# julius-speech/julius

Hardware: AMD Instinct MI355X
Metric: frames_x_states_scored_per_sec (higher is better)
Workload: dtype f32; 1 GPU; C2 = configs[1]: triphone GMM outprob only, S=3000 M=16 D=39, step = 12 launches x 64000 frames; frames_per_launch=64000, parallelism=utterance-sharded x1, kernel=gmm_tile<D=39,FPL=2,NS=16,ring> grid=23504 nsb=16

## Files before the change

### julius_amd/csrc/gmm_api.hip

```cpp
#include "gmm_host.h"

extern "C" {

int jamd_gmm_create(jamd_engine *e, const jamd_gmm_desc *d, int gprune, int gprune_num, jamd_gmm **out) {
  if (!e || !d || !out) { jamd_set_error("jamd_gmm_create: NULL argument"); return JAMD_EINVAL; }
  *out = nullptr;
  if (d->nstream != 1) {
    jamd_set_error("jamd_gmm_create: nstream=%d; only single-stream models are supported", d->nstream);
    return JAMD_EINVAL;
  }
  if (d->nstate <= 0 || d->veclen <= 0 || d->veclen > 1024 || d->nentry < 0 || d->ndens < 0) {
    jamd_set_error("jamd_gmm_create: bad dimensions S=%d D=%d G=%d E=%d", d->nstate, d->veclen,
                   d->ndens, d->nentry);
    return JAMD_EINVAL;
  }
  if (gprune != JAMD_GPRUNE_NONE && gprune != JAMD_GPRUNE_SAFE && gprune != JAMD_GPRUNE_HEU && gprune != JAMD_GPRUNE_BEAM) {
    jamd_set_error("jamd_gmm_create: unknown gprune method %d", gprune);
    return JAMD_EINVAL;
  }
  const bool history_pruning = gprune == JAMD_GPRUNE_HEU || gprune == JAMD_GPRUNE_BEAM;
  const int requested_gprune = gprune;
  if (history_pruning) gprune = JAMD_GPRUNE_SAFE;
  if (!d->mean || !d->ivar || !d->gconst || !d->st_off || (d->nentry && (!d->ent_dens || !d->ent_logw))) {
    jamd_set_error("jamd_gmm_create: NULL model array");
    return JAMD_EINVAL;
  }
  if (d->st_off[0] != 0 || d->st_off[d->nstate] != d->nentry) {
    jamd_set_error("jamd_gmm_create: st_off must run from 0 to nentry");
    return JAMD_EINVAL;
  }
  JAMD_HIP(hipSetDevice(e->device));
  std::unique_ptr<jamd_gmm> g(new jamd_gmm());
  int rc;
  g->eng = e; g->S = d->nstate; g->D = d->veclen; g->E = d->nentry;
  g->gprune = gprune; g->gprune_num = gprune_num;
  const int D = g->D;
  g->rec = ((2 * D + 2) + 3) & ~3;
  const bool have_books = d->nbook > 0 && d->st_book;
  std::vector<int> st_off_plain(g->S + 1, 0), tied;
  std::vector<int> book_first(d->nbook > 0 ? d->nbook : 0, -1);
  for (int s = 0; s < g->S; s++) {
    const int n = d->st_off[s + 1] - d->st_off[s];
    if (n < 0) { jamd_set_error("jamd_gmm_create: st_off not monotone at %d", s); return JAMD_EINVAL; }
    const int b = have_books ? d->st_book[s] : -1;
    if (b >= d->nbook) { jamd_set_error("jamd_gmm_create: codebook id %d out of range", b); return JAMD_EINVAL; }
    if (b >= 0) {
      tied.push_back(s);
      if (book_first[b] < 0) book_first[b] = s;
      else if (n != d->st_off[book_first[b] + 1] - d->st_off[book_first[b]]) {
        jamd_set_error("jamd_gmm_create: states of codebook %d disagree on its size", b); return JAMD_EINVAL;
      }
      st_off_plain[s + 1] = st_off_plain[s];
    } else {
      if (n > g->maxmix) g->maxmix = n;
      st_off_plain[s + 1] = st_off_plain[s] + n;
    }
  }
  g->E_plain = st_off_plain[g->S];
  g->ntied = (int)tied.size();
  if (history_pruning && g->ntied > 0) g->hist_method = requested_gprune;
  g->nbook = g->ntied ? d->nbook : 0;
  if (gprune == JAMD_GPRUNE_SAFE && gprune_num < 1) {
    jamd_set_error("jamd_gmm_create: gprune safe needs gprune_num >= 1"); return JAMD_EINVAL;
  }
  if (gprune == JAMD_GPRUNE_SAFE && gprune_num > 64) {
    jamd_set_error("jamd_gmm_create: gprune_num %d > 64 is not supported on the device", gprune_num);
    return JAMD_EINVAL;
  }
  auto fill_rec = [&](float *r, int dn, float lw) -> bool {
    if (dn >= d->ndens) return false;
    if (dn >= 0) {
      memcpy(r, d->mean + (size_t)dn * D, sizeof(float) * D);
      memcpy(r + D, d->ivar + (size_t)dn * D, sizeof(float) * D);
      r[2 * D] = d->gconst[dn];
      if (r[2 * D] != r[2 * D]) g->has_null = true;
    } else {
      r[2 * D] = __builtin_nanf("");
      g->has_null = true;
    }
    r[2 * D + 1] = lw;
    return true;
  };
  std::vector<float> rec((size_t)g->E_plain * g->rec, 0.0f);
  for (int s = 0; s < g->S; s++) {
    if (have_books && d->st_book[s] >= 0) continue;
    for (int k = 0; k < d->st_off[s + 1] - d->st_off[s]; k++) {
      const int en = d->st_off[s] + k;
      if (!fill_rec(rec.data() + (size_t)(st_off_plain[s] + k) * g->rec, d->ent_dens[en], d->ent_logw[en])) {
        jamd_set_error("jamd_gmm_create: density index %d out of range", d->ent_dens[en]); return JAMD_EINVAL;
      }
    }
  }
  if ((rc = g->d_rec.upload(rec.data(), rec.size())) != JAMD_OK) return rc;
  if (D == 39) {
    constexpr int kRing = 80;
    std::vector<float> ring((size_t)g->E_plain * kRing, 0.0f);
    for (int en = 0; en < g->E_plain; en++) {
      const float *r = rec.data() + (size_t)en * g->rec;
      float *q = ring.data() + (size_t)en * kRing;
      q[0] = r[2 * D]; q[1] = r[2 * D + 1];
      for (int k = 0; k < 7; k++) { q[2 + k] = r[k]; q[9 + k] = r[D + k]; }
      for (int c = 1; c < 5; c++)
        for (int k = 0; k < 8; k++) { q[16 * c + k] = r[8 * c - 1 + k]; q[16 * c + 8 + k] = r[D + 8 * c - 1 + k]; }
    }
    if ((rc = g->d_rec_ring.upload(ring.data(), ring.size())) != JAMD_OK) return rc;
  }
  if ((rc = g->d_st_off.upload(d->st_off, g->S + 1)) != JAMD_OK) return rc;
  if ((rc = g->d_st_off_plain.upload(st_off_plain.data(), g->S + 1)) != JAMD_OK) return rc;
  if (g->ntied) {
    std::vector<int> book_off(g->nbook + 1, 0);
    for (int b = 0; b < g->nbook; b++) {
      const int n = book_first[b] >= 0 ? d->st_off[book_first[b] + 1] - d->st_off[book_first[b]] : 0;
      book_off[b + 1] = book_off[b] + n;
      if (n > g->maxbook) g->maxbook = n;
    }
    std::vector<float> brec((size_t)book_off[g->nbook] * g->rec, 0.0f);
    for (int b = 0; b < g->nbook; b++) {
      if (book_first[b] < 0) continue;
      for (int k = 0; k < book_off[b + 1] - book_off[b]; k++) {
        if (!fill_rec(brec.data() + (size_t)(book_off[b] + k) * g->rec,
                      d->ent_dens[d->st_off[book_first[b]] + k], 0.0f)) {
          jamd_set_error("jamd_gmm_create: codebook density index out of range"); return JAMD_EINVAL;
        }
      }
    }
    g->tm_cap = (gprune == JAMD_GPRUNE_NONE) ? g->maxbook : (gprune_num < g->maxbook ? gprune_num : g->maxbook);
    g->h_book_off = book_off;
    if ((rc = g->d_book_rec.upload(brec.data(), brec.size())) != JAMD_OK) return rc;
    if ((rc = g->d_book_off.upload(book_off.data(), g->nbook + 1)) != JAMD_OK) return rc;
    if ((rc = g->d_st_book.upload(d->st_book, g->S)) != JAMD_OK) return rc;
    if ((rc = g->d_ent_logw.upload(d->ent_logw, g->E)) != JAMD_OK) return rc;
    if ((rc = g->d_tied_states.upload(tied.data(), g->ntied)) != JAMD_OK) return rc;
  }
  *out = g.release();
  return JAMD_OK;
}

void jamd_gmm_destroy(jamd_gmm *g) {
  if (!g) return;
  (void)hipSetDevice(g->eng->device);
  delete g;
}

int jamd_gmm_nstate(const jamd_gmm *g) { return g ? g->S : -1; }
int jamd_gmm_veclen(const jamd_gmm *g) { return g ? g->D : -1; }
const char *jamd_gmm_last_kernel(const jamd_gmm *g) { return g ? g->last_kernel : ""; }

int jamd_gmm_nentry(const jamd_gmm *g) {
  if (!g) return 0;
  if (g->ntied == 0) return g->E;
  if (g->ntied == g->S && !g->h_book_off.empty()) return g->h_book_off[g->nbook];
  return 0;
}

int jamd_gmm_book_offsets(const jamd_gmm *g, int *off, int cap) {
  if (!g || !off || g->ntied != g->S || (int)g->h_book_off.size() != g->nbook + 1 || cap < g->nbook + 1) {
    jamd_set_error("jamd_gmm_book_offsets: not an all-tied-mixture model, or buffer too small"); return JAMD_EINVAL;
  }
  memcpy(off, g->h_book_off.data(), sizeof(int) * (size_t)(g->nbook + 1));
  return JAMD_OK;
}

int jamd_gmm_dens_dev(jamd_gmm *g, const float *dev_frames, int T, float *dev_out, void *stream) {
  if (!g || !dev_frames || !dev_out || T < 0) { jamd_set_error("jamd_gmm_dens_dev: bad argument"); return JAMD_EINVAL; }
  const int E = jamd_gmm_nentry(g);
  if (E <= 0) {
    jamd_set_error("jamd_gmm_dens_dev: models mixing plain and tied-mixture states have no single column order");
    return JAMD_EINVAL;
  }
  if (T == 0) return JAMD_OK;
  JAMD_HIP(hipSetDevice(g->eng->device));
  hipStream_t st = jamd_stream(g->eng, stream);
  const int rc = jamd_gmm_launch_dens(g, g->ntied ? g->d_book_rec : g->d_rec, E, dev_frames, T, dev_out, st);
  if (rc != JAMD_OK) return rc;
  hipError_t le = hipGetLastError();
  if (le != hipSuccess) { jamd_set_error("jamd_gmm_dens_dev: launch failed: %s", hipGetErrorString(le)); return JAMD_ELAUNCH; }
  return JAMD_OK;
}

int jamd_gmm_dens_host(jamd_gmm *g, const float *host_frames, int T, float *host_out) {
  if (!g || !host_frames || !host_out || T < 0) { jamd_set_error("jamd_gmm_dens_host: bad argument"); return JAMD_EINVAL; }
  if (T == 0) return JAMD_OK;
  JAMD_HIP(hipSetDevice(g->eng->device));
  const int E = jamd_gmm_nentry(g);
  if (E <= 0) { jamd_set_error("jamd_gmm_dens_host: no single column order for this model"); return JAMD_EINVAL; }
  return jamd_host_call(&g->dens_stage, g->eng, host_frames, (size_t)T * g->D, host_out, (size_t)T * E,
                        [&](const float *in, float *o, hipStream_t st) -> long long {
                          const int rc = jamd_gmm_dens_dev(g, in, T, o, st);
                          return rc != JAMD_OK ? rc : (long long)T * E;
                        }, JAMD_ELAUNCH);
}

static int set_utterances(jamd_gmm *g, const int *utt_off, int nutt, hipStream_t st) {
  if (g->ntied == 0 || g->gprune == JAMD_GPRUNE_NONE) return JAMD_OK;
  const size_t bytes = sizeof(int) * ((size_t)nutt + 1);
  int rc;
  if ((rc = g->utt.begin(bytes < 4096 ? 4096 : bytes)) != JAMD_OK) return rc;
  memcpy(g->utt.h.p, utt_off, bytes);
  if ((rc = g->utt.send(bytes, st)) != JAMD_OK) return rc;
  g->cur_nutt = nutt;
  return JAMD_OK;
}

int jamd_gmm_outprob_dev(jamd_gmm *g, const float *dev_frames, int T, float *dev_out, void *stream) {
  const int off[2] = {0, T};
  if (T < 0) { jamd_set_error("jamd_gmm_outprob_dev: bad argument"); return JAMD_EINVAL; }
  return jamd_gmm_outprob_utts_dev(g, dev_frames, off, 1, dev_out, stream);
}

int jamd_gmm_outprob_utts_dev(jamd_gmm *g, const float *dev_frames, const int *utt_off, int nutt, float *dev_out, void *stream) {
  if (!g || !dev_frames || !dev_out || !utt_off || nutt < 1 || utt_off[0] != 0) {
    jamd_set_error("jamd_gmm_outprob_utts_dev: bad argument");
    return JAMD_EINVAL;
  }
  for (int u = 0; u < nutt; u++)
    if (utt_off[u + 1] < utt_off[u]) { jamd_set_error("jamd_gmm_outprob_utts_dev: utt_off must be non-decreasing"); return JAMD_EINVAL; }
  const int T = utt_off[nutt];
  if (T == 0) return JAMD_OK;
  JAMD_HIP(hipSetDevice(g->eng->device));
  hipStream_t st = jamd_stream(g->eng, stream);
  int rc = JAMD_OK;
  if ((rc = set_utterances(g, utt_off, nutt, st)) != JAMD_OK) return rc;
  if (g->E_plain == 0 && g->ntied == g->S) {
  } else if (g->gprune == JAMD_GPRUNE_SAFE) {
    rc = jamd_gmm_launch_safe(g, dev_frames, T, dev_out, st);
  } else {
    rc = jamd_gmm_launch_plain(g, dev_frames, T, dev_out, st);
  }
  if (rc != JAMD_OK) return rc;
  if (g->ntied) {
    const size_t n = (size_t)T * g->nbook * g->tm_cap;
    if ((rc = g->d_tm_score.grow(sizeof(float) * n)) != JAMD_OK) return rc;
    if ((rc = g->d_tm_id.grow(sizeof(int) * n)) != JAMD_OK) return rc;
    if ((rc = g->d_tm_num.grow(sizeof(int) * (size_t)T * g->nbook)) != JAMD_OK) return rc;
    if ((rc = jamd_gmm_launch_tmix(g, dev_frames, T, dev_out, g->d_tm_score, g->d_tm_id, g->d_tm_num, st)) != JAMD_OK) return rc;
  }
  hipError_t le = hipGetLastError();
  if (le != hipSuccess) {
    jamd_set_error("jamd_gmm_outprob_dev: launch failed: %s", hipGetErrorString(le));
    return JAMD_ELAUNCH;
  }
  return JAMD_OK;
}

int jamd_gmm_outprob_host(jamd_gmm *g, const float *host_frames, int T, float *host_out) {
  if (!g || !host_frames || !host_out || T < 0) {
    jamd_set_error("jamd_gmm_outprob_host: bad argument");
    return JAMD_EINVAL;
  }
  if (T == 0) return JAMD_OK;
  return jamd_host_call(&g->stage, g->eng, host_frames, (size_t)T * g->D, host_out, (size_t)T * g->S,
                        [&](const float *in, float *o, hipStream_t st) -> long long {
                          const int rc = jamd_gmm_outprob_dev(g, in, T, o, st);
                          return rc != JAMD_OK ? rc : (long long)T * g->S;
                        }, JAMD_ELAUNCH);
}

int jamd_gmm_tmix_cap(const jamd_gmm *g) { return g ? g->tm_cap : -1; }
int jamd_gmm_nbook(const jamd_gmm *g) { return g ? g->nbook : -1; }

int jamd_gmm_tmix_cache_dev(jamd_gmm *g, const float *dev_frames, int T, float *dev_score,
                            int *dev_id, int *dev_num, void *stream) {
  if (!g || !dev_frames || !dev_score || !dev_id || !dev_num || T < 0) {
    jamd_set_error("jamd_gmm_tmix_cache_dev: bad argument");
    return JAMD_EINVAL;
  }
  if (!g->ntied) { jamd_set_error("jamd_gmm_tmix_cache_dev: model has no tied-mixture states"); return JAMD_ESTATE; }
  if (T == 0) return JAMD_OK;
  JAMD_HIP(hipSetDevice(g->eng->device));
  const int off[2] = {0, T};
  int rc = set_utterances(g, off, 1, jamd_stream(g->eng, stream));
  if (rc == JAMD_OK) rc = jamd_gmm_launch_tmix(g, dev_frames, T, nullptr, dev_score, dev_id, dev_num, jamd_stream(g->eng, stream));
  if (rc != JAMD_OK) return rc;
  hipError_t le = hipGetLastError();
  if (le != hipSuccess) {
    jamd_set_error("jamd_gmm_tmix_cache_dev: launch failed: %s", hipGetErrorString(le));
    return JAMD_ELAUNCH;
  }
  return JAMD_OK;
}

}
```

### julius_amd/csrc/gmm_host.h

```cpp
#pragma once
#include "jamd_host.h"

struct JAMD_LOCAL jamd_gmm {
  jamd_engine *eng = nullptr;
  int S = 0, D = 0, E = 0, nbook = 0;
  int gprune = 0, gprune_num = 0;
  int rec = 0;
  int maxmix = 0;
  JamdDev<float> d_rec;
  JamdDev<float> d_rec_ring;
  JamdDev<int> d_st_off;
  JamdDev<int> d_st_off_plain;
  int E_plain = 0;
  JamdDev<int> d_st_book;
  JamdDev<int> d_book_off;
  std::vector<int> h_book_off;
  JamdDev<float> d_book_rec;
  JamdDev<float> d_ent_logw;
  JamdDev<int> d_tied_states;
  int ntied = 0;
  int maxbook = 0;
  int tm_cap = 0;
  bool has_null = false;
  int hist_method = 0;
  JamdPinned utt;
  int cur_nutt = 0;
  JamdStage<float, float> stage;
  JamdStage<float, float> dens_stage;
  JamdDev<float> d_tm_score; JamdDev<int> d_tm_id, d_tm_num;
  JamdDev<float> d_narrow;
  JamdDev<int> d_tm_flag;
  char last_kernel[64] = {0};
};

JAMD_LOCAL int jamd_gmm_launch_plain(jamd_gmm *g, const float *frames, int T, float *out, hipStream_t st);
JAMD_LOCAL int jamd_gmm_launch_dens(jamd_gmm *g, const float *rec, int E, const float *frames, int T, float *out,
                                        hipStream_t st);

int jamd_gmm_launch_safe(jamd_gmm *g, const float *frames, int T, float *out, hipStream_t st);
int jamd_gmm_launch_tmix(jamd_gmm *g, const float *frames, int T, float *out, float *c_score,
                         int *c_id, int *c_num, hipStream_t st);
```

### julius_amd/csrc/gmm_outprob.hip

```cpp
#include "gmm_dev.h"
#include "gmm_host.h"

namespace {
using namespace jamd;

constexpr int kWaves = 4;

template <int D, int FPL, int NS, bool HAS_NULL>
__global__ void __launch_bounds__(64 * kWaves)
gmm_tile_kernel(const float *__restrict__ rec, const int *__restrict__ st_off,
                const float *__restrict__ frames, const float *__restrict__ tbl,
                float *__restrict__ out, int T, int S, int nsb, int nfb, int nstb,
                float addmin_f) {
  static_assert(FPL % 2 == 0, "frames are processed as packed pairs");
  constexpr int REC = ((2 * D + 2) + 3) & ~3;
  constexpr int FPW = 64 * FPL;
  constexpr int NP = FPL / 2;
  __shared__ float tile[kWaves][FPW][NS + 1];

  int fb, sb;
  if (!decode_block(nfb, nstb, fb, sb)) return;
  const int lane = threadIdx.x & 63;
  const int wave = threadIdx.x >> 6;
  const int t0 = (fb * kWaves + wave) * FPW;
  if (t0 >= T) return;

  f2 v[NP][D];
#pragma unroll
  for (int p = 0; p < NP; p++) load_frames<D>(v[p], nullptr, frames, t0 + p * 128, T, D, lane);

#if defined(__HIP_DEVICE_COMPILE__) && !defined(__GFX9__)
#error "gmm_tile: the raw buffer descriptor below is the gfx9 (CDNA) format; this library is written for gfx950 only"
#endif
  const __amdgpu_buffer_rsrc_t tbl_rsrc = __builtin_amdgcn_make_buffer_rsrc((void *)tbl, 0, 4 * (JAMD_TBLSIZE + 1), 0x00020000);
  const int s_begin = sb * nsb;
  const int s_end = min(S, s_begin + nsb);
  for (int sg = s_begin; sg < s_end; sg += NS) {
    const int ns = min(NS, s_end - sg);
    for (int si = 0; si < ns; si++) {
      const int e0 = st_off[sg + si], e1 = st_off[sg + si + 1];
      f2 y2[NP], tv2[NP];
#pragma unroll
      for (int p = 0; p < NP; p++) { y2[p] = f2{JAMD_LOG_ZERO, JAMD_LOG_ZERO}; tv2[p] = f2{0.0f, 0.0f}; }
      for (int e = e1 - 1; e >= e0; e--) {
        const float *__restrict__ r = rec + (size_t)e * REC;
        const float gc = r[2 * D], lw = r[2 * D + 1];
        f2 acc[NP];
#pragma unroll
        for (int p = 0; p < NP; p++) acc[p] = f2{gc, gc};
#pragma unroll
        for (int d = 0; d < D; d++) {
          const float mu = r[d], iv = r[D + d];
          const f2 mu2 = {mu, mu}, iv2 = {iv, iv};
#pragma unroll
          for (int p = 0; p < NP; p++) {
            f2 x = v[p][d] - mu2;
            x = x * x;
            x = x * iv2;
            acc[p] = acc[p] + x;
          }
        }
        const bool nulld = HAS_NULL && (gc != gc);
        const float naddmin = -addmin_f;
#pragma unroll
        for (int p = 0; p < NP; p++) {
          f2 s2 = acc[p] * f2{-0.5f, -0.5f};
          if (nulld) s2 = f2{JAMD_LOG_ZERO, JAMD_LOG_ZERO};
          s2 = s2 + f2{lw, lw};
          __builtin_amdgcn_sched_barrier(0);
          const f2 yy = y2[p] + tv2[p];
          const f2 hi = {__builtin_fmaxf(s2.x, yy.x), __builtin_fmaxf(s2.y, yy.y)};
          const f2 df = s2 - yy;
          const float a0 = __builtin_fabsf(df.x), a1 = __builtin_fabsf(df.y);
          unsigned o0 = ((unsigned)((double)a0 * JAMD_TMAG + 0.5)) << 2, o1 = ((unsigned)((double)a1 * JAMD_TMAG + 0.5)) << 2;
          o0 = (a0 <= naddmin) ? o0 : 4u * (unsigned)JAMD_TBLSIZE;
          o1 = (a1 <= naddmin) ? o1 : 4u * (unsigned)JAMD_TBLSIZE;
          tv2[p] = f2{__builtin_bit_cast(float, __builtin_amdgcn_raw_buffer_load_b32(tbl_rsrc, (int)o0, 0, 0)),
                      __builtin_bit_cast(float, __builtin_amdgcn_raw_buffer_load_b32(tbl_rsrc, (int)o1, 0, 0))};
          y2[p] = hi;
        }
      }
#pragma unroll
      for (int k = 0; k < FPL; k++) {
        const f2 fin = y2[k / 2] + tv2[k / 2];
        tile[wave][k * 64 + lane][si] = finish_state((k & 1) ? fin.y : fin.x);
      }
    }
    wave_sync();
    constexpr int RPI = 64 / NS;
    const int col = lane % NS, rsub = lane / NS;
#pragma unroll 4
    for (int it = 0; it < FPW / RPI; it++) {
      const int rr = it * RPI + rsub;
      const int t = t0 + rr;
      if (t < T && col < ns) out[(size_t)t * S + sg + col] = tile[wave][rr][col];
    }
    wave_release();
  }
}

typedef float f16v __attribute__((ext_vector_type(16)));
constexpr int kRingRec = 80;

template <int BYTE_OFF>
__device__ __forceinline__ void ring_load(f16v &home, const float *chunks) {
  __builtin_amdgcn_sched_barrier(0);
  asm volatile("s_load_dwordx16 %0, %1, %2" : "=s"(home) : "s"(chunks), "i"(BYTE_OFF));
  __builtin_amdgcn_sched_barrier(0);
}
__device__ __forceinline__ void ring_wait(f16v &h0, f16v &h1, f16v &h2) {
  __builtin_amdgcn_sched_barrier(0);
  asm volatile("s_waitcnt lgkmcnt(0)" : "+s"(h0), "+s"(h1), "+s"(h2));
  __builtin_amdgcn_sched_barrier(0);
}
template <int N, int MU0, int IV0>
__device__ __forceinline__ void ring_chunk(f2 &acc, const f2 *v, const f16v &h) {
  f2 x[N], q[N], w[N];
#pragma unroll
  for (int i = 0; i < N + 3; i++) {
    if (i < N) { const float mu = h[MU0 + i]; x[i] = v[i] - f2{mu, mu}; }
    if (i >= 1 && i - 1 < N) q[i - 1] = x[i - 1] * x[i - 1];
    if (i >= 2 && i - 2 < N) { const float iv = h[IV0 + i - 2]; w[i - 2] = q[i - 2] * f2{iv, iv}; }
    if (i >= 3) acc = acc + w[i - 3];
    __builtin_amdgcn_sched_barrier(0);
  }
}

template <int NS, bool HAS_NULL>
__global__ void __launch_bounds__(64 * kWaves)
gmm_tile_ring_kernel(const float *__restrict__ ring, const int *__restrict__ st_off,
                     const float *__restrict__ frames, const float *__restrict__ tbl,
                     float *__restrict__ out, int T, int S, int nsb, int nfb, int nstb,
                     float addmin_f) {
  constexpr int D = 39, FPL = 2;
  constexpr int FPW = 64 * FPL;
  __shared__ float tile[kWaves][FPW][NS + 1];

  int fb, sb;
  if (!decode_block(nfb, nstb, fb, sb)) return;
  const int lane = threadIdx.x & 63;
  const int wave = threadIdx.x >> 6;
  const int t0 = (fb * kWaves + wave) * FPW;
  if (t0 >= T) return;

  f2 v[D];
  load_frames<D>(v, nullptr, frames, t0, T, D, lane);

  const __amdgpu_buffer_rsrc_t tbl_rsrc = __builtin_amdgcn_make_buffer_rsrc((void *)tbl, 0, 4 * (JAMD_TBLSIZE + 1), 0x00020000);
  const float naddmin = -addmin_f;
  const int s_begin = sb * nsb;
  const int s_end = min(S, s_begin + nsb);
  f16v h0, h1, h2;
  int held = -1;
  for (int sg = s_begin; sg < s_end; sg += NS) {
    const int ns = min(NS, s_end - sg);
    for (int si = 0; si < ns; si++) {
      const int s = sg + si;
      const int e0 = st_off[s], e1 = st_off[s + 1];
      const int e_over = (s + 1 < s_end ? st_off[s + 2] : e1) - 1;
      f2 y2 = {JAMD_LOG_ZERO, JAMD_LOG_ZERO}, tv2 = {0.0f, 0.0f};
      if (e1 > e0 && held != e1 - 1) {
        const float *r = ring + (size_t)(e1 - 1) * kRingRec;
        ring_load<0>(h0, r);
        ring_load<64>(h1, r);
        ring_load<128>(h2, r);
        ring_wait(h0, h1, h2);
      }
      for (int e = e1 - 1; e >= e0; e--) {
        const float *r = ring + (size_t)e * kRingRec;
        const float *rn = ring + (size_t)(e > e0 ? e - 1 : e_over) * kRingRec;
        const float gc = h0[0], lw = h0[1];
        const bool nulld = HAS_NULL && (gc != gc);
        f2 acc = {gc, gc};
        ring_chunk<7, 2, 9>(acc, v, h0);
        ring_load<192>(h0, r);
        ring_chunk<8, 0, 8>(acc, v + 7, h1);
        ring_load<256>(h1, r);
        ring_chunk<8, 0, 8>(acc, v + 15, h2);
        ring_wait(h0, h1, h2);
        ring_chunk<8, 0, 8>(acc, v + 23, h0);
        ring_load<0>(h0, rn);
        ring_load<128>(h2, rn);
        ring_chunk<8, 0, 8>(acc, v + 31, h1);
        ring_load<64>(h1, rn);
        {
          f2 s2 = acc * f2{-0.5f, -0.5f};
          if (nulld) s2 = f2{JAMD_LOG_ZERO, JAMD_LOG_ZERO};
          s2 = s2 + f2{lw, lw};
          __builtin_amdgcn_sched_barrier(0);
          const f2 yy = y2 + tv2;
          const f2 hi = {__builtin_fmaxf(s2.x, yy.x), __builtin_fmaxf(s2.y, yy.y)};
          const f2 df = s2 - yy;
          const float a0 = __builtin_fabsf(df.x), a1 = __builtin_fabsf(df.y);
          unsigned o0 = ((unsigned)((double)a0 * JAMD_TMAG + 0.5)) << 2, o1 = ((unsigned)((double)a1 * JAMD_TMAG + 0.5)) << 2;
          o0 = (a0 <= naddmin) ? o0 : 4u * (unsigned)JAMD_TBLSIZE;
          o1 = (a1 <= naddmin) ? o1 : 4u * (unsigned)JAMD_TBLSIZE;
          tv2 = f2{__builtin_bit_cast(float, __builtin_amdgcn_raw_buffer_load_b32(tbl_rsrc, (int)o0, 0, 0)),
                   __builtin_bit_cast(float, __builtin_amdgcn_raw_buffer_load_b32(tbl_rsrc, (int)o1, 0, 0))};
          y2 = hi;
        }
        ring_wait(h0, h1, h2);
      }
      if (e1 > e0) held = e_over;
      const f2 fin = y2 + tv2;
      tile[wave][lane][si] = finish_state(fin.x);
      tile[wave][64 + lane][si] = finish_state(fin.y);
    }
    store_tile<NS, FPW>(tile[wave], out, t0, T, S, sg, ns, lane);
  }
}

template <int FPL, int NS>
__global__ void __launch_bounds__(64 * kWaves)
gmm_tile_generic_kernel(const float *__restrict__ rec, const int *__restrict__ st_off,
                        const float *__restrict__ frames, const float *__restrict__ tbl,
                        float *__restrict__ out, int T, int S, int D, int REC, int nsb, int nfb,
                        int nstb, float addmin_f) {
  static_assert(FPL == 2, "load_frames / gauss_pair hold one packed pair of frames per lane");
  constexpr int FPW = 64 * FPL;
  __shared__ float tile[kWaves][FPW][NS + 1];
  extern __shared__ __align__(16) float dyn[];

  int fb, sb;
  if (!decode_block(nfb, nstb, fb, sb)) return;
  const int lane = threadIdx.x & 63;
  const int wave = threadIdx.x >> 6;
  const int t0 = (fb * kWaves + wave) * FPW;
  if (t0 >= T) return;
  float *vt = dyn + (size_t)wave * D * FPW;
  load_frames<0>(nullptr, vt, frames, t0, T, D, lane);

  const int s_begin = sb * nsb;
  const int s_end = min(S, s_begin + nsb);
  for (int sg = s_begin; sg < s_end; sg += NS) {
    const int ns = min(NS, s_end - sg);
    for (int si = 0; si < ns; si++) {
      const int e0 = st_off[sg + si], e1 = st_off[sg + si + 1];
      float y0 = JAMD_LOG_ZERO, y1 = JAMD_LOG_ZERO;
      for (int e = e1 - 1; e >= e0; e--) {
        const float *__restrict__ r = rec + (size_t)e * REC;
        const float lw = r[2 * D + 1];
        const f2 g = gauss_pair<0>(nullptr, vt, lane, D, r);
        y0 = addlog_step(y0, g.x + lw, tbl, addmin_f);
        y1 = addlog_step(y1, g.y + lw, tbl, addmin_f);
      }
      tile[wave][lane][si] = finish_state(y0);
      tile[wave][64 + lane][si] = finish_state(y1);
    }
    store_tile<NS, FPW>(tile[wave], out, t0, T, S, sg, ns, lane);
  }
}

template <int D, int FPL, int NS>
int launch_tile(jamd_gmm *g, const float *frames, int T, float *out, hipStream_t st) {
  constexpr int FPB = kWaves * 64 * FPL;
  const int nfb = (T + FPB - 1) / FPB;
  const int nsb = NS;
  const int nstb = (g->S + nsb - 1) / nsb;
  const int grid = xcd_grid(nstb, nfb);
  if constexpr (D == 39 && FPL == 2) {
    if (g->has_null)
      hipLaunchKernelGGL((gmm_tile_ring_kernel<NS, true>), dim3(grid), dim3(64 * kWaves), 0, st,
                         g->d_rec_ring, g->d_st_off_plain, frames, g->eng->d_addlog, out, T, g->S, nsb, nfb,
                         nstb, g->eng->addmin_f);
    else
      hipLaunchKernelGGL((gmm_tile_ring_kernel<NS, false>), dim3(grid), dim3(64 * kWaves), 0, st,
                         g->d_rec_ring, g->d_st_off_plain, frames, g->eng->d_addlog, out, T, g->S, nsb, nfb,
                         nstb, g->eng->addmin_f);
    snprintf(g->last_kernel, sizeof(g->last_kernel), "gmm_tile<D=%d,FPL=%d,NS=%d,ring> grid=%d nsb=%d", D, FPL, NS, grid, nsb);
  } else {
    if (g->has_null)
      hipLaunchKernelGGL((gmm_tile_kernel<D, FPL, NS, true>), dim3(grid), dim3(64 * kWaves), 0, st,
                         g->d_rec, g->d_st_off_plain, frames, g->eng->d_addlog, out, T, g->S, nsb, nfb,
                         nstb, g->eng->addmin_f);
    else
      hipLaunchKernelGGL((gmm_tile_kernel<D, FPL, NS, false>), dim3(grid), dim3(64 * kWaves), 0, st,
                         g->d_rec, g->d_st_off_plain, frames, g->eng->d_addlog, out, T, g->S, nsb, nfb,
                         nstb, g->eng->addmin_f);
    snprintf(g->last_kernel, sizeof(g->last_kernel), "gmm_tile<D=%d,FPL=%d,NS=%d> grid=%d nsb=%d", D, FPL, NS, grid, nsb);
  }
  return JAMD_OK;
}

template <int FPL, int NS>
int launch_tile_generic(jamd_gmm *g, const float *frames, int T, float *out, hipStream_t st) {
  constexpr int FPB = kWaves * 64 * FPL;
  const int nfb = (T + FPB - 1) / FPB;
  const int nsb = NS;
  const int nstb = (g->S + nsb - 1) / nsb;
  const int grid = xcd_grid(nstb, nfb);
  const size_t dyn = sizeof(float) * kWaves * g->D * 64 * FPL;
  const int rc = jamd_reserve_dyn_lds((const void *)gmm_tile_generic_kernel<FPL, NS>, dyn, "GMM outprob");
  if (rc != JAMD_OK) return rc;
  hipLaunchKernelGGL((gmm_tile_generic_kernel<FPL, NS>), dim3(grid), dim3(64 * kWaves), dyn, st,
                     g->d_rec, g->d_st_off_plain, frames, g->eng->d_addlog, out, T, g->S, g->D, g->rec,
                     nsb, nfb, nstb, g->eng->addmin_f);
  snprintf(g->last_kernel, sizeof(g->last_kernel), "gmm_tile_generic<FPL=%d,NS=%d> D=%d grid=%d",
           FPL, NS, g->D, grid);
  return JAMD_OK;
}

constexpr int kNarrowT = 256;
constexpr int kNarrowFB = 8;
template <int D, bool HAS_NULL>
__global__ void __launch_bounds__(64)
gmm_narrow_dens_kernel(const float *__restrict__ rec, const float *__restrict__ frames, float *__restrict__ dens, int T, int E,
                       int nfb, int neb) {
  constexpr int REC = (2 * D + 2 + 3) & ~3;
  int fbk, ebk;
  if (!decode_block(nfb, neb, fbk, ebk)) return;
  const int e = ebk * 64 + threadIdx.x;
  const float4 *__restrict__ r4 = reinterpret_cast<const float4 *>(rec + (size_t)(e < E ? e : E - 1) * REC);
  float r[REC];
#pragma unroll
  for (int q = 0; q < REC / 4; q++) { const float4 v = r4[q]; r[4 * q] = v.x; r[4 * q + 1] = v.y; r[4 * q + 2] = v.z; r[4 * q + 3] = v.w; }
  const float gc = r[2 * D], lw = r[2 * D + 1];
  const bool nulld = HAS_NULL && (gc != gc);
  const int t_end = min(T, (fbk + 1) * kNarrowFB);
  for (int t = fbk * kNarrowFB; t < t_end; t += 2) {
    const float *__restrict__ fa = frames + (size_t)t * D;
    const float *__restrict__ fb = frames + (size_t)(t + 1 < T ? t + 1 : t) * D;
    f2 acc = {gc, gc};
#pragma unroll
    for (int d = 0; d < D; d++) {
      f2 x = f2{fa[d], fb[d]} - f2{r[d], r[d]};
      x = x * x;
      x = x * f2{r[D + d], r[D + d]};
      acc = acc + x;
    }
    f2 s2 = acc * f2{-0.5f, -0.5f};
    if (nulld) s2 = f2{JAMD_LOG_ZERO, JAMD_LOG_ZERO};
    s2 = s2 + f2{lw, lw};
    if (e < E) {
      dens[(size_t)t * E + e] = s2.x;
      if (t + 1 < T) dens[(size_t)(t + 1) * E + e] = s2.y;
    }
  }
}

__global__ void __launch_bounds__(256)
gmm_narrow_lse_kernel(const float *__restrict__ dens, const int *__restrict__ st_off, const float *__restrict__ tbl,
                      float *__restrict__ out, int T, int S, int E, float addmin_f) {
  const int i = blockIdx.x * 256 + threadIdx.x;
  if (i >= T * S) return;
  const int t = i / S, s = i - t * S;
  const int e0 = st_off[s], e1 = st_off[s + 1];
  const float *__restrict__ dr = dens + (size_t)t * E;
  float y = JAMD_LOG_ZERO;
  int e = e1 - 1;
  for (; e - 7 >= e0; e -= 8) {
    float v[8];
#pragma unroll
    for (int q = 0; q < 8; q++) v[q] = dr[e - q];
#pragma unroll
    for (int q = 0; q < 8; q++) y = addlog_step(y, v[q], tbl, addmin_f);
  }
  for (; e >= e0; e--) y = addlog_step(y, dr[e], tbl, addmin_f);
  out[(size_t)t * S + s] = finish_state(y);
}

template <int D>
int launch_narrow(jamd_gmm *g, const float *frames, int T, float *out, hipStream_t st) {
  const int E = g->E_plain;
  int rc = g->d_narrow.grow(sizeof(float) * (size_t)kNarrowT * (size_t)E);
  if (rc != JAMD_OK) return rc;
  const int grid = (E + 63) / 64;
  const int nfb = (T + kNarrowFB - 1) / kNarrowFB;
  const dim3 gr(xcd_grid(grid, nfb));
  if (g->has_null) hipLaunchKernelGGL((gmm_narrow_dens_kernel<D, true>), gr, dim3(64), 0, st, g->d_rec, frames, g->d_narrow, T, E, nfb, grid);
  else hipLaunchKernelGGL((gmm_narrow_dens_kernel<D, false>), gr, dim3(64), 0, st, g->d_rec, frames, g->d_narrow, T, E, nfb, grid);
  hipLaunchKernelGGL(gmm_narrow_lse_kernel, dim3((T * g->S + 255) / 256), dim3(256), 0, st, g->d_narrow, g->d_st_off_plain,
                     g->eng->d_addlog, out, T, g->S, E, g->eng->addmin_f);
  snprintf(g->last_kernel, sizeof(g->last_kernel), "gmm_narrow<D=%d> grid=%d + lse", D, grid);
  return JAMD_OK;
}

constexpr int kDensChunk = 1024;
__global__ void __launch_bounds__(64)
gmm_dens_kernel(const float *__restrict__ rec, const float *__restrict__ frames, float *__restrict__ out,
                int T, int E, int D, int REC) {
  extern __shared__ float xs[];
  float (*tile)[17] = reinterpret_cast<float (*)[17]>(xs + (size_t)D * 64);
  const int lane = threadIdx.x;
  const int t0 = blockIdx.x * 64, e_begin = blockIdx.y * kDensChunk;
  const int e_end = min(E, e_begin + kDensChunk);
  {
    int t = t0 + lane; if (t > T - 1) t = T - 1;
    const float *f = frames + (size_t)t * D;
    for (int d = 0; d < D; d++) xs[d * 64 + lane] = f[d];
  }
  wave_sync();
  for (int e0 = e_begin; e0 < e_end; e0 += 16) {
    const int ne = min(16, e_end - e0);
    for (int g = 0; g < ne; g++) {
      const float *__restrict__ r = rec + (size_t)(e0 + g) * REC;
      const float gc = r[2 * D];
      float acc = gc;
      for (int d = 0; d < D; d++) {
        float x = xs[d * 64 + lane] - r[d];
        x = x * x;
        x = x * r[D + d];
        acc = acc + x;
      }
      float sc = acc * -0.5f;
      if (gc != gc) sc = JAMD_LOG_ZERO;
      tile[lane][g] = sc;
    }
    wave_sync();
    const int col = lane & 15, rsub = lane >> 4;
    for (int it = 0; it < 16; it++) {
      const int rr = it * 4 + rsub, t = t0 + rr;
      if (t < T && col < ne) out[(size_t)t * E + e0 + col] = tile[rr][col];
    }
    wave_release();
  }
}

}


int jamd_gmm_launch_plain(jamd_gmm *g, const float *frames, int T, float *out, hipStream_t st) {
  const bool narrow = T <= kNarrowT && g->E_plain > 0;
  return dispatch_veclen(g->D, [&](auto dt) {
    constexpr int D = decltype(dt)::value;
    if constexpr (D == 0) return launch_tile_generic<2, 16>(g, frames, T, out, st);
    else return narrow ? launch_narrow<D>(g, frames, T, out, st) : launch_tile<D, 2, 16>(g, frames, T, out, st);
  });
}

int jamd_gmm_launch_dens(jamd_gmm *g, const float *rec, int E, const float *frames, int T, float *out, hipStream_t st) {
  const size_t lds = sizeof(float) * ((size_t)g->D * 64 + 64 * 17);
  if (lds > 64 * 1024) { jamd_set_error("jamd_gmm_dens_dev: vector length %d too large", g->D); return JAMD_EINVAL; }
  hipLaunchKernelGGL(gmm_dens_kernel, dim3((T + 63) / 64, (E + kDensChunk - 1) / kDensChunk), dim3(64), lds, st,
                     rec, frames, out, T, E, g->D, g->rec);
  return JAMD_OK;
}
```

Before: 19.78 billion frame*states/s.

## Add persistent pull-based work distribution to the D=39 ring GMM kernel

Adds a persistent variant of the ring GMM tile kernel. It launches roughly one occupancy-sized grid instead of one block per tile. Each wave pulls (state-range, frame-group) tickets from eight atomic counters spread across cache lines, using a deal that keeps state-range locality per share. The aim is to cut block launch and tail-imbalance overhead on large launches, at the cost of per-ticket atomics, a memset before each launch and reloading frames per ticket. The path is chosen when the tile count exceeds a multiple of the pull grid capacity, and environment variables can override that threshold and the grid size.

```diff
diff --git a/julius_amd/csrc/gmm_api.hip b/julius_amd/csrc/gmm_api.hip
--- a/julius_amd/csrc/gmm_api.hip
+++ b/julius_amd/csrc/gmm_api.hip
@@ -104,6 +104,7 @@
         for (int k = 0; k < 8; k++) { q[16 * c + k] = r[8 * c - 1 + k]; q[16 * c + 8 + k] = r[D + 8 * c - 1 + k]; }
     }
     if ((rc = g->d_rec_ring.upload(ring.data(), ring.size())) != JAMD_OK) return rc;
+    if ((rc = jamd_gmm_pull_setup(g.get())) != JAMD_OK) return rc;
   }
   if ((rc = g->d_st_off.upload(d->st_off, g->S + 1)) != JAMD_OK) return rc;
   if ((rc = g->d_st_off_plain.upload(st_off_plain.data(), g->S + 1)) != JAMD_OK) return rc;
diff --git a/julius_amd/csrc/gmm_deal.h b/julius_amd/csrc/gmm_deal.h
--- /dev/null
+++ b/julius_amd/csrc/gmm_deal.h
@@ -0,0 +1,57 @@
+#pragma once
+
+#if defined(__HIPCC__)
+#define GD_HD __host__ __device__ inline __attribute__((always_inline))
+#else
+#define GD_HD inline
+#endif
+
+constexpr int kGdShares = 8;
+constexpr int kGdHeadStride = 32;
+
+struct GmmDeal {
+  int nfw;
+  int k8;
+  int full;
+  int L, per;
+};
+
+GD_HD GmmDeal gd_make(int nstb, int nfw) {
+  GmmDeal d;
+  d.nfw = nfw;
+  d.k8 = nstb & ~7;
+  d.full = (d.k8 >> 3) * nfw;
+  d.L = (nstb - d.k8) * nfw;
+  d.per = (d.L + 7) >> 3;
+  return d;
+}
+
+GD_HD int gd_len(const GmmDeal &d, int x) {
+  int left = d.L - x * d.per;
+  if (left < 0) left = 0;
+  if (left > d.per) left = d.per;
+  return d.full + left;
+}
+
+GD_HD bool gd_ticket(const GmmDeal &d, int x, int n, int &range, int &group) {
+  if (n < 0) return false;
+  if (n < d.full) {
+    const int q = n / d.nfw;
+    range = x + 8 * q;
+    group = n - q * d.nfw;
+    return true;
+  }
+  const int k = n - d.full;
+  if (k >= d.per) return false;
+  const int m = x * d.per + k;
+  if (m >= d.L) return false;
+  const int q = m / d.nfw;
+  range = d.k8 + q;
+  group = m - q * d.nfw;
+  return true;
+}
+
+GD_HD int gd_pull_grid(int cap, int want) {
+  int g = (want > 0 ? want : cap) & ~7;
+  return g < 8 ? 8 : g;
+}
diff --git a/julius_amd/csrc/gmm_host.h b/julius_amd/csrc/gmm_host.h
--- a/julius_amd/csrc/gmm_host.h
+++ b/julius_amd/csrc/gmm_host.h
@@ -30,10 +30,15 @@
   JamdDev<float> d_tm_score; JamdDev<int> d_tm_id, d_tm_num;
   JamdDev<float> d_narrow;
   JamdDev<int> d_tm_flag;
+  JamdDev<int> d_pull_heads;
+  int pull_cap = 0;
+  int pull_min = 0;
+  int pull_grid = 0;
   char last_kernel[64] = {0};
 };
 
 JAMD_LOCAL int jamd_gmm_launch_plain(jamd_gmm *g, const float *frames, int T, float *out, hipStream_t st);
+JAMD_LOCAL int jamd_gmm_pull_setup(jamd_gmm *g);
 JAMD_LOCAL int jamd_gmm_launch_dens(jamd_gmm *g, const float *rec, int E, const float *frames, int T, float *out,
                                         hipStream_t st);
 
diff --git a/julius_amd/csrc/gmm_outprob.hip b/julius_amd/csrc/gmm_outprob.hip
--- a/julius_amd/csrc/gmm_outprob.hip
+++ b/julius_amd/csrc/gmm_outprob.hip
@@ -1,5 +1,6 @@
 #include "gmm_dev.h"
 #include "gmm_host.h"
+#include "gmm_deal.h"
 
 namespace {
 using namespace jamd;
@@ -126,87 +127,110 @@
   }
 }
 
-template <int NS, bool HAS_NULL>
+template <int NS, bool HAS_NULL, bool PULL>
 __global__ void __launch_bounds__(64 * kWaves)
 gmm_tile_ring_kernel(const float *__restrict__ ring, const int *__restrict__ st_off,
                      const float *__restrict__ frames, const float *__restrict__ tbl,
                      float *__restrict__ out, int T, int S, int nsb, int nfb, int nstb,
-                     float addmin_f) {
+                     float addmin_f, int *__restrict__ heads) {
   constexpr int D = 39, FPL = 2;
   constexpr int FPW = 64 * FPL;
   __shared__ float tile[kWaves][FPW][NS + 1];
 
-  int fb, sb;
-  if (!decode_block(nfb, nstb, fb, sb)) return;
   const int lane = threadIdx.x & 63;
   const int wave = threadIdx.x >> 6;
-  const int t0 = (fb * kWaves + wave) * FPW;
-  if (t0 >= T) return;
-
   f2 v[D];
-  load_frames<D>(v, nullptr, frames, t0, T, D, lane);
+  int sb, t0;
+  if constexpr (!PULL) {
+    int fb;
+    if (!decode_block(nfb, nstb, fb, sb)) return;
+    t0 = (fb * kWaves + wave) * FPW;
+    if (t0 >= T) return;
+    load_frames<D>(v, nullptr, frames, t0, T, D, lane);
+  }
 
   const __amdgpu_buffer_rsrc_t tbl_rsrc = __builtin_amdgcn_make_buffer_rsrc((void *)tbl, 0, 4 * (JAMD_TBLSIZE + 1), 0x00020000);
   const float naddmin = -addmin_f;
-  const int s_begin = sb * nsb;
-  const int s_end = min(S, s_begin + nsb);
+  int share = blockIdx.x & (kGdShares - 1), spent = 0;
   f16v h0, h1, h2;
   int held = -1;
-  for (int sg = s_begin; sg < s_end; sg += NS) {
-    const int ns = min(NS, s_end - sg);
-    for (int si = 0; si < ns; si++) {
-      const int s = sg + si;
-      const int e0 = st_off[s], e1 = st_off[s + 1];
-      const int e_over = (s + 1 < s_end ? st_off[s + 2] : e1) - 1;
-      f2 y2 = {JAMD_LOG_ZERO, JAMD_LOG_ZERO}, tv2 = {0.0f, 0.0f};
-      if (e1 > e0 && held != e1 - 1) {
-        const float *r = ring + (size_t)(e1 - 1) * kRingRec;
-        ring_load<0>(h0, r);
-        ring_load<64>(h1, r);
-        ring_load<128>(h2, r);
-        ring_wait(h0, h1, h2);
-      }
-      for (int e = e1 - 1; e >= e0; e--) {
-        const float *r = ring + (size_t)e * kRingRec;
-        const float *rn = ring + (size_t)(e > e0 ? e - 1 : e_over) * kRingRec;
-        const float gc = h0[0], lw = h0[1];
-        const bool nulld = HAS_NULL && (gc != gc);
-        f2 acc = {gc, gc};
-        ring_chunk<7, 2, 9>(acc, v, h0);
-        ring_load<192>(h0, r);
-        ring_chunk<8, 0, 8>(acc, v + 7, h1);
-        ring_load<256>(h1, r);
-        ring_chunk<8, 0, 8>(acc, v + 15, h2);
-        ring_wait(h0, h1, h2);
-        ring_chunk<8, 0, 8>(acc, v + 23, h0);
-        ring_load<0>(h0, rn);
-        ring_load<128>(h2, rn);
-        ring_chunk<8, 0, 8>(acc, v + 31, h1);
-        ring_load<64>(h1, rn);
-        {
-          f2 s2 = acc * f2{-0.5f, -0.5f};
-          if (nulld) s2 = f2{JAMD_LOG_ZERO, JAMD_LOG_ZERO};
-          s2 = s2 + f2{lw, lw};
-          __builtin_amdgcn_sched_barrier(0);
-          const f2 yy = y2 + tv2;
-          const f2 hi = {__builtin_fmaxf(s2.x, yy.x), __builtin_fmaxf(s2.y, yy.y)};
-          const f2 df = s2 - yy;
-          const float a0 = __builtin_fabsf(df.x), a1 = __builtin_fabsf(df.y);
-          unsigned o0 = ((unsigned)((double)a0 * JAMD_TMAG + 0.5)) << 2, o1 = ((unsigned)((double)a1 * JAMD_TMAG + 0.5)) << 2;
-          o0 = (a0 <= naddmin) ? o0 : 4u * (unsigned)JAMD_TBLSIZE;
-          o1 = (a1 <= naddmin) ? o1 : 4u * (unsigned)JAMD_TBLSIZE;
-          tv2 = f2{__builtin_bit_cast(float, __builtin_amdgcn_raw_buffer_load_b32(tbl_rsrc, (int)o0, 0, 0)),
-                   __builtin_bit_cast(float, __builtin_amdgcn_raw_buffer_load_b32(tbl_rsrc, (int)o1, 0, 0))};
-          y2 = hi;
+  for (;;) {
+    if constexpr (PULL) {
+      const GmmDeal deal = gd_make(nstb, nfb);
+      int group = 0;
+      bool got = false;
+      while (spent < kGdShares) {
+        int n = 0;
+        if (lane == 0) n = __hip_atomic_fetch_add(heads + share * kGdHeadStride, 1, __ATOMIC_RELAXED, __HIP_MEMORY_SCOPE_AGENT);
+        n = __builtin_amdgcn_readfirstlane(n);
+        got = gd_ticket(deal, share, n, sb, group);
+        if (got) break;
+        share = (share + 1) & (kGdShares - 1);
+        spent++;
+      }
+      if (!got) return;
+      t0 = group * FPW;
+      load_frames<D>(v, nullptr, frames, t0, T, D, lane);
+    }
+    const int s_begin = sb * nsb;
+    const int s_end = min(S, s_begin + nsb);
+    for (int sg = s_begin; sg < s_end; sg += NS) {
+      const int ns = min(NS, s_end - sg);
+      for (int si = 0; si < ns; si++) {
+        const int s = sg + si;
+        const int e0 = st_off[s], e1 = st_off[s + 1];
+        const int e_over = (s + 1 < s_end ? st_off[s + 2] : e1) - 1;
+        f2 y2 = {JAMD_LOG_ZERO, JAMD_LOG_ZERO}, tv2 = {0.0f, 0.0f};
+        if (e1 > e0 && held != e1 - 1) {
+          const float *r = ring + (size_t)(e1 - 1) * kRingRec;
+          ring_load<0>(h0, r);
+          ring_load<64>(h1, r);
+          ring_load<128>(h2, r);
+          ring_wait(h0, h1, h2);
         }
-        ring_wait(h0, h1, h2);
-      }
-      if (e1 > e0) held = e_over;
-      const f2 fin = y2 + tv2;
-      tile[wave][lane][si] = finish_state(fin.x);
-      tile[wave][64 + lane][si] = finish_state(fin.y);
-    }
-    store_tile<NS, FPW>(tile[wave], out, t0, T, S, sg, ns, lane);
+        for (int e = e1 - 1; e >= e0; e--) {
+          const float *r = ring + (size_t)e * kRingRec;
+          const float *rn = ring + (size_t)(e > e0 ? e - 1 : e_over) * kRingRec;
+          const float gc = h0[0], lw = h0[1];
+          const bool nulld = HAS_NULL && (gc != gc);
+          f2 acc = {gc, gc};
+          ring_chunk<7, 2, 9>(acc, v, h0);
+          ring_load<192>(h0, r);
+          ring_chunk<8, 0, 8>(acc, v + 7, h1);
+          ring_load<256>(h1, r);
+          ring_chunk<8, 0, 8>(acc, v + 15, h2);
+          ring_wait(h0, h1, h2);
+          ring_chunk<8, 0, 8>(acc, v + 23, h0);
+          ring_load<0>(h0, rn);
+          ring_load<128>(h2, rn);
+          ring_chunk<8, 0, 8>(acc, v + 31, h1);
+          ring_load<64>(h1, rn);
+          {
+            f2 s2 = acc * f2{-0.5f, -0.5f};
+            if (nulld) s2 = f2{JAMD_LOG_ZERO, JAMD_LOG_ZERO};
+            s2 = s2 + f2{lw, lw};
+            __builtin_amdgcn_sched_barrier(0);
+            const f2 yy = y2 + tv2;
+            const f2 hi = {__builtin_fmaxf(s2.x, yy.x), __builtin_fmaxf(s2.y, yy.y)};
+            const f2 df = s2 - yy;
+            const float a0 = __builtin_fabsf(df.x), a1 = __builtin_fabsf(df.y);
+            unsigned o0 = ((unsigned)((double)a0 * JAMD_TMAG + 0.5)) << 2, o1 = ((unsigned)((double)a1 * JAMD_TMAG + 0.5)) << 2;
+            o0 = (a0 <= naddmin) ? o0 : 4u * (unsigned)JAMD_TBLSIZE;
+            o1 = (a1 <= naddmin) ? o1 : 4u * (unsigned)JAMD_TBLSIZE;
+            tv2 = f2{__builtin_bit_cast(float, __builtin_amdgcn_raw_buffer_load_b32(tbl_rsrc, (int)o0, 0, 0)),
+                     __builtin_bit_cast(float, __builtin_amdgcn_raw_buffer_load_b32(tbl_rsrc, (int)o1, 0, 0))};
+            y2 = hi;
+          }
+          ring_wait(h0, h1, h2);
+        }
+        if (e1 > e0) held = e_over;
+        const f2 fin = y2 + tv2;
+        tile[wave][lane][si] = finish_state(fin.x);
+        tile[wave][64 + lane][si] = finish_state(fin.y);
+      }
+      store_tile<NS, FPW>(tile[wave], out, t0, T, S, sg, ns, lane);
+    }
+    if constexpr (!PULL) break;
   }
 }
 
@@ -251,6 +275,10 @@
   }
 }
 
+constexpr int kNarrowT = 256;
+constexpr int kPullNS = 16;
+constexpr int kPullRounds = 8;
+
 template <int D, int FPL, int NS>
 int launch_tile(jamd_gmm *g, const float *frames, int T, float *out, hipStream_t st) {
   constexpr int FPB = kWaves * 64 * FPL;
@@ -259,14 +287,30 @@
   const int nstb = (g->S + nsb - 1) / nsb;
   const int grid = xcd_grid(nstb, nfb);
   if constexpr (D == 39 && FPL == 2) {
+    static_assert(NS == kPullNS, "jamd_gmm_pull_setup() asks the occupancy of this instantiation");
+    if (g->pull_min >= 0 && T > kNarrowT && (long long)nstb * nfb > g->pull_min) {
+      const int nfw = (T + 64 * FPL - 1) / (64 * FPL);
+      const int pgrid = gd_pull_grid(g->pull_cap, g->pull_grid);
+      JAMD_HIP(hipMemsetAsync(g->d_pull_heads, 0, sizeof(int) * kGdShares * kGdHeadStride, st));
+      if (g->has_null)
+        hipLaunchKernelGGL((gmm_tile_ring_kernel<NS, true, true>), dim3(pgrid), dim3(64 * kWaves), 0, st,
+                           g->d_rec_ring, g->d_st_off_plain, frames, g->eng->d_addlog, out, T, g->S, nsb, nfw,
+                           nstb, g->eng->addmin_f, g->d_pull_heads);
+      else
+        hipLaunchKernelGGL((gmm_tile_ring_kernel<NS, false, true>), dim3(pgrid), dim3(64 * kWaves), 0, st,
+                           g->d_rec_ring, g->d_st_off_plain, frames, g->eng->d_addlog, out, T, g->S, nsb, nfw,
+                           nstb, g->eng->addmin_f, g->d_pull_heads);
+      snprintf(g->last_kernel, sizeof(g->last_kernel), "gmm_tile<D=%d,FPL=%d,NS=%d,ring,pull> grid=%d nsb=%d", D, FPL, NS, pgrid, nsb);
+      return JAMD_OK;
+    }
     if (g->has_null)
-      hipLaunchKernelGGL((gmm_tile_ring_kernel<NS, true>), dim3(grid), dim3(64 * kWaves), 0, st,
+      hipLaunchKernelGGL((gmm_tile_ring_kernel<NS, true, false>), dim3(grid), dim3(64 * kWaves), 0, st,
                          g->d_rec_ring, g->d_st_off_plain, frames, g->eng->d_addlog, out, T, g->S, nsb, nfb,
-                         nstb, g->eng->addmin_f);
+                         nstb, g->eng->addmin_f, (int *)nullptr);
     else
-      hipLaunchKernelGGL((gmm_tile_ring_kernel<NS, false>), dim3(grid), dim3(64 * kWaves), 0, st,
+      hipLaunchKernelGGL((gmm_tile_ring_kernel<NS, false, false>), dim3(grid), dim3(64 * kWaves), 0, st,
                          g->d_rec_ring, g->d_st_off_plain, frames, g->eng->d_addlog, out, T, g->S, nsb, nfb,
-                         nstb, g->eng->addmin_f);
+                         nstb, g->eng->addmin_f, (int *)nullptr);
     snprintf(g->last_kernel, sizeof(g->last_kernel), "gmm_tile<D=%d,FPL=%d,NS=%d,ring> grid=%d nsb=%d", D, FPL, NS, grid, nsb);
   } else {
     if (g->has_null)
@@ -300,7 +344,6 @@
   return JAMD_OK;
 }
 
-constexpr int kNarrowT = 256;
 constexpr int kNarrowFB = 8;
 template <int D, bool HAS_NULL>
 __global__ void __launch_bounds__(64)
@@ -419,6 +462,20 @@
 }
 
 
+int jamd_gmm_pull_setup(jamd_gmm *g) {
+  if (g->D != 39) return JAMD_OK;
+  int rc, per_cu = 0;
+  if ((rc = g->d_pull_heads.alloc(kGdShares * kGdHeadStride, true)) != JAMD_OK) return rc;
+  if (g->has_null) JAMD_HIP(hipOccupancyMaxActiveBlocksPerMultiprocessor(&per_cu, gmm_tile_ring_kernel<kPullNS, true, true>, 64 * kWaves, 0));
+  else JAMD_HIP(hipOccupancyMaxActiveBlocksPerMultiprocessor(&per_cu, gmm_tile_ring_kernel<kPullNS, false, true>, 64 * kWaves, 0));
+  g->pull_cap = (per_cu * g->eng->num_cu) & ~7;
+  if (g->pull_cap < 8) g->pull_cap = 8;
+  g->pull_min = kPullRounds * g->pull_cap;
+  if (const char *s = getenv("JAMD_GMM_PULL_MIN")) g->pull_min = atoi(s);
+  if (const char *s = getenv("JAMD_GMM_PULL_GRID")) g->pull_grid = atoi(s);
+  return JAMD_OK;
+}
+
 int jamd_gmm_launch_plain(jamd_gmm *g, const float *frames, int T, float *out, hipStream_t st) {
   const bool narrow = T <= kNarrowT && g->E_plain > 0;
   return dispatch_veclen(g->D, [&](auto dt) {
```

Result: faster. 20.36 billion frame*states/s (median of 6 runs) (+3.0%).
